# PaullyMac/routest

Measured on AMD Instinct MI355X. Metric: ETA preds/sec (whole node) + p50 /predict latency, 3-layer MLP bf16, higher is better.
Workload: dtype bf16

## Files before the change

### csrc/cch_bindings.cpp

```cpp
#include <torch/extension.h>
#include <ATen/hip/impl/HIPStreamMasqueradingAsCUDA.h>
#include <c10/core/DeviceGuard.h>

#include <chrono>
#include <cmath>
#include <memory>
#include <mutex>
#include <unordered_map>

#include "cch_gpu.h"
#include "ops.h"

namespace py = pybind11;

namespace {

#define CCH_CHECK_HIP(expr)                                                            \
  do {                                                                                 \
    hipError_t _e = (expr);                                                            \
    TORCH_CHECK(_e == hipSuccess, "HIP error in ", #expr, ": ", hipGetErrorString(_e)); \
  } while (0)

hipStream_t stream_of(int dev) { return c10::hip::getCurrentHIPStreamMasqueradingAsCUDA(dev).stream(); }

// ... 267 lines not shown
    o.path = want_path ? path.data_ptr<int>() : nullptr;
    o.max_path = (int)max_path;
    const c10::DeviceGuard guard(src.device());
    std::lock_guard<std::mutex> lk(mu_);
    CCH_CHECK_HIP(g_->route(*m, src.data_ptr<int>(), dst.data_ptr<int>(), (int)Q, o, *sc_, stream_of(dev_)));
    return py::make_tuple(sec, met, st, len, path);
  }

  py::tuple matrix(int64_t key, torch::Tensor pts, torch::Tensor npts) {
    auto m = get(key);
    TORCH_CHECK(pts.is_cuda() && npts.is_cuda() && pts.dim() == 2 && pts.scalar_type() == torch::kInt32 &&
                    npts.scalar_type() == torch::kInt32 && npts.numel() == pts.size(0) && pts.is_contiguous(),
                "pts int32 [R, NM], npts int32 [R] on the router's GPU");
    const int R = (int)pts.size(0), NM = (int)pts.size(1);
    auto of = torch::TensorOptions().dtype(torch::kFloat32).device(torch::kCUDA, dev_);
    auto sec = torch::empty({R, NM, NM}, of), met = torch::empty({R, NM, NM}, of);
    const c10::DeviceGuard guard(pts.device());
    std::lock_guard<std::mutex> lk(mu_);
    CCH_CHECK_HIP(g_->matrix(*m, pts.data_ptr<int>(), npts.data_ptr<int>(), R, NM, sec.data_ptr<float>(),
                             met.data_ptr<float>(), nullptr, *sc_, stream_of(dev_)));
    return py::make_tuple(sec, met);
  }

  py::tuple matrix_rect(int64_t key, torch::Tensor src, torch::Tensor nsrc, torch::Tensor dst, torch::Tensor ndst,
                        int64_t meet) {
    auto m = get(key);
    for (const torch::Tensor* t : {&src, &nsrc, &dst, &ndst})
      TORCH_CHECK(t->is_cuda() && t->device().index() == dev_ && t->scalar_type() == torch::kInt32 && t->is_contiguous(),
                  "src / nsrc / dst / ndst: int32 on the router's GPU");
    TORCH_CHECK(src.dim() == 2 && dst.dim() == 2 && dst.size(0) == src.size(0) && nsrc.numel() == src.size(0) &&
                    ndst.numel() == src.size(0),
                "src [R, SM], dst [R, DM], nsrc [R], ndst [R]");
    const int64_t R = src.size(0), SM = src.size(1), DM = dst.size(1);
    TORCH_CHECK(R * (SM + DM) <= INT32_MAX && R * SM * DM <= INT32_MAX, "matrix_rect: too many chains or cells for one call");
    auto of = torch::TensorOptions().dtype(torch::kFloat32).device(torch::kCUDA, dev_);
    auto sec = torch::empty({R, SM, DM}, of), met = torch::empty({R, SM, DM}, of);
    const c10::DeviceGuard guard(src.device());
    std::lock_guard<std::mutex> lk(mu_);
    CCH_CHECK_HIP(g_->matrix_rect(*m, src.data_ptr<int>(), nsrc.data_ptr<int>(), dst.data_ptr<int>(),
                                  ndst.data_ptr<int>(), (int)R, (int)SM, (int)DM, sec.data_ptr<float>(),
                                  met.data_ptr<float>(), *sc_, stream_of(dev_), (int)meet));
    return py::make_tuple(sec, met);
  }

  py::tuple matrix_keep(int64_t key, torch::Tensor pts, torch::Tensor npts) {
    auto sm = matrix(key, pts, npts);
// ... 107 lines not shown

}

void bind_cch_gpu(py::module& m) {
  py::class_<PyCchGpu>(m, "CchGpu")
      .def(py::init<torch::Tensor, torch::Tensor, torch::Tensor, torch::Tensor, torch::Tensor, torch::Tensor,
                    torch::Tensor, int64_t>(),
           py::arg("indptr"), py::arg("indices"), py::arg("lat"), py::arg("lon"), py::arg("length"),
           py::arg("road_class"), py::arg("base_traffic"), py::arg("device"))
      .def("set_eta", &PyCchGpu::set_eta, py::arg("blob"), py::arg("H"), py::arg("norm"), py::arg("variant") = -1)
      .def("stats", &PyCchGpu::stats)
      .def("metric_for", &PyCchGpu::metric_for, py::arg("weather"), py::arg("congestion"), py::arg("weekhour"),
           py::arg("driver_age") = 35.0, py::arg("pin") = false, py::arg("avoid") = py::none(),
           py::arg("avoid_digest") = 0)
      .def("avoid_mask", &PyCchGpu::avoid_mask, py::arg("blob"))
      .def("unpin", &PyCchGpu::unpin, py::arg("key"))
      .def("pinned", &PyCchGpu::pinned)
      .def("metric_from_costs", &PyCchGpu::metric_from_costs, py::arg("key"), py::arg("cost"))
      .def("costs", &PyCchGpu::costs, py::arg("key"))
      .def("metric_dump", &PyCchGpu::metric_dump, py::arg("key"))
      .def("route", &PyCchGpu::route, py::arg("key"), py::arg("src"), py::arg("dst"), py::arg("max_path") = 4096,
           py::arg("want_path") = true)
      .def("matrix", &PyCchGpu::matrix, py::arg("key"), py::arg("pts"), py::arg("npts"))
      .def("matrix_rect", &PyCchGpu::matrix_rect, py::arg("key"), py::arg("src"), py::arg("nsrc"), py::arg("dst"),
           py::arg("ndst"), py::arg("meet") = 0)
      .def("matrix_keep", &PyCchGpu::matrix_keep, py::arg("key"), py::arg("pts"), py::arg("npts"))
      .def("legs_from_matrix", &PyCchGpu::legs_from_matrix, py::arg("key"), py::arg("tag"), py::arg("pts"), py::arg("r"),
           py::arg("i"), py::arg("j"), py::arg("max_path") = 4096, py::arg("want_path") = true)
      .def("one_to_all", &PyCchGpu::one_to_all, py::arg("key"), py::arg("src"), py::arg("reverse") = false,
           py::arg("fuse") = -1)
      .def("set_capacity", &PyCchGpu::set_capacity)
      .def("set_cache_gb", &PyCchGpu::set_cache_gb, py::arg("gb"))
      .def("set_builder_pacing", &PyCchGpu::set_builder_pacing, py::arg("max_workgroups"), py::arg("always") = false)
      .def("set_unpack_serial", &PyCchGpu::set_unpack_serial, py::arg("on"))
      .def("unpack_serial", &PyCchGpu::unpack_serial)
      .def("request_build", &PyCchGpu::request_build, py::arg("weather"), py::arg("congestion"), py::arg("weekhour"),
           py::arg("driver_age") = 35.0, py::arg("urgent") = true, py::arg("avoid") = py::none(),
           py::arg("avoid_digest") = 0)
      .def("is_cached", &PyCchGpu::is_cached, py::arg("key"))
      .def("ptr", &PyCchGpu::ptr)
      .def("topology_arrays", &PyCchGpu::topology_arrays);
}
```

### csrc/cch_gpu.h

```cpp
#pragma once
#include <hip/hip_runtime.h>

#include <cstdint>
#include <cstdlib>
#include <cstring>
#include <atomic>
#include <chrono>
#include <condition_variable>
#include <deque>
#include <functional>
#include <list>
#include <memory>
#include <mutex>
#include <thread>
#include <unordered_set>
#include <vector>

#include "common.h"
#include "runtime/cch.h"

namespace rt {

struct CchContext {
  int weather = 2, congestion = 1, weekhour = 9;
// ... 22 lines not shown
  int4* b_rec = nullptr;
  int64_t kept_f = 0, kept_b = 0;
  double customize_ms = 0.0, cost_ms = 0.0;
  double basic_ms = 0.0, perfect_ms = 0.0, prune_ms = 0.0;
  double alloc_ms = 0.0, hostcopy_ms = 0.0;
  std::vector<float> host_cost;
  std::shared_ptr<const std::vector<int32_t>> avoid;
  ~CchMetricDev();
};

struct CchScratch {
  float* dist = nullptr;
  int32_t* pred = nullptr;
  int32_t* node = nullptr;
  size_t jobs_cap = 0;
  int32_t* jobs = nullptr;
  int32_t* arcs = nullptr;
  int32_t* narcs = nullptr;
  size_t pairs_cap = 0;
  int32_t* pj = nullptr;
  size_t pj_cap = 0;
  uint64_t chain_tag = 0;
  int chain_nm = 0, chain_r = 0;
  int device = 0;
  std::vector<void*> old;
  ~CchScratch();
  hipError_t ensure(size_t jobs, size_t pairs, int stride, int max_arcs);
};

struct CchAllScratch {
  float* sec = nullptr;
  float* met = nullptr;
  size_t blocks_cap = 0;
  int device = 0;
  std::vector<void*> old;
  ~CchAllScratch();
  hipError_t ensure(size_t blocks, size_t N);
};

struct CustScratch {
  unsigned long long *up64 = nullptr, *dn64 = nullptr;
  uint32_t *pup = nullptr, *pdn = nullptr;
  int32_t *fcnt = nullptr, *bcnt = nullptr;
  void* cub = nullptr;
  size_t cub_bytes = 0;
  void* rec_buf = nullptr;
  float* min_buf = nullptr;
  float* h_stage = nullptr;
  unsigned long long* sup_buf = nullptr;
  int32_t* avoid_dev = nullptr;
// ... 64 lines not shown
  double cache_gb() { std::lock_guard<std::mutex> lk(mu_); return cache_gb_; }
  int capacity() { std::lock_guard<std::mutex> lk(mu_); return capacity_; }
  int64_t metric_bytes() const { return metric_bytes_.load(); }
  int cached() { std::lock_guard<std::mutex> lk(mu_); return (int)cache_.size(); }

  void request_build(const CchContext& c, bool urgent = true);
  void start_builders();
  int add_build_listener(std::function<void(uint64_t, bool)> cb);
  void remove_build_listener(int id);
  struct AsyncStats {
    long long queued = 0, built = 0, failed = 0;
    int pending = 0;
    double build_ms = 0.0, alloc_ms = 0.0, hostcopy_ms = 0.0;
    long long paced = 0;
  };
  AsyncStats async_stats();
  void set_builder_pacing(int n, bool always = false) {
    builder_max_wg_.store(n < 0 ? 0 : n);
    pace_always_.store(always);
  }
  int builder_pacing() const { return builder_max_wg_.load(); }
  void set_unpack_serial(bool on) { unpack_serial_.store(on); }
  bool unpack_serial() const { return unpack_serial_.load(); }
  void note_queries() {
    query_us_.store(std::chrono::duration_cast<std::chrono::microseconds>(
                        std::chrono::steady_clock::now().time_since_epoch()).count(),
                    std::memory_order_relaxed);
  }
  bool serving_now() const {
    const long long now = std::chrono::duration_cast<std::chrono::microseconds>(
                              std::chrono::steady_clock::now().time_since_epoch()).count();
    return now - query_us_.load(std::memory_order_relaxed) < 250000;
  }

  hipError_t route(const CchMetricDev& m, const int* d_src, const int* d_dst, int Q, const CchRouteOut& o,
                   CchScratch& sc, hipStream_t s);
  hipError_t matrix(const CchMetricDev& m, const int* d_pts, const int* d_npts, int R, int NM, float* d_sec,
                    float* d_met, double* d_D64, CchScratch& sc, hipStream_t s);
  hipError_t legs_from_matrix(const CchMetricDev& m, const int* d_src, const int* d_r, const int* d_i, const int* d_j,
                              int Q, uint64_t tag, const CchRouteOut& o, CchScratch& sc, hipStream_t s);
  static constexpr int MAX_ARCS = 1024;
  enum { MEET_AUTO = 0, MEET_RECT = 1, MEET_PAIRS = 2, MEET_NONE = 3 };
  hipError_t matrix_rect(const CchMetricDev& m, const int* d_src, const int* d_nsrc, const int* d_dst,
                         const int* d_ndst, int R, int SM, int DM, float* d_sec, float* d_met, CchScratch& sc,
                         hipStream_t s, int meet = MEET_AUTO);

// ... 1 lines not shown
                        CchAllScratch& sc, hipStream_t s, int fuse = -1);
  static constexpr size_t ALL_SCRATCH_BYTES = 1ull << 30;
  static constexpr int ALL_FUSE_WIDTH = 4;

  static CchMView view(const CchMetricDev& m) {
    return CchMView{m.f_ptr, m.b_ptr, m.f_rec, m.b_rec, m.len_up, m.len_dn, m.sub_up, m.sub_dn, m.cnt_up, m.cnt_dn};
  }
  hipError_t route_multi(const CchMView* d_mv, const int* d_grp, const int* d_src, const int* d_dst, int Q,
                         const CchRouteOut& o, CchScratch& sc, hipStream_t s);
  hipError_t matrix_multi(const CchMView* d_mv, const int* d_row_grp, const int* d_pts, const int* d_npts, int R, int NM,
                          float* d_sec, float* d_met, double* d_D64, CchScratch& sc, hipStream_t s);
  hipError_t legs_from_matrix_multi(const CchMView* d_mv, const int* d_grp, const int* d_src, const int* d_r,
                                    const int* d_i, const int* d_j, int Q, uint64_t tag, const CchRouteOut& o,
                                    CchScratch& sc, hipStream_t s);

 private:
  hipError_t route_impl(const CchMetricDev* m, const CchMView* mv, const int* grp, const int* d_src, const int* d_dst,
                        int Q, const CchRouteOut& o, CchScratch& sc, hipStream_t s);
  hipError_t matrix_impl(const CchMetricDev* m, const CchMView* mv, const int* grp, const int* d_pts, const int* d_npts,
                         int R, int NM, float* d_sec, float* d_met, double* d_D64, CchScratch& sc, hipStream_t s);
  hipError_t legs_impl(const CchMetricDev* m, const CchMView* mv, const int* grp, const int* d_src, const int* d_r,
                       const int* d_i, const int* d_j, int Q, uint64_t tag, const CchRouteOut& o, CchScratch& sc,
                       hipStream_t s);
  hipError_t launch_unpack(const CchMetricDev* m, const CchMView* mv, const int* grp, int Q, const int* d_src,
                           CchScratch& sc, const CchRouteOut& o, hipStream_t s);
  rcch::Topology T_;
  int dev_ = 0;
  int32_t *d_up_ptr = nullptr, *d_up_head = nullptr, *d_arc_lo = nullptr, *d_parent = nullptr, *d_depth = nullptr;
  int32_t *d_rank = nullptr, *d_node = nullptr, *d_edge_arc = nullptr;
  uint8_t* d_edge_dir = nullptr;
  float* d_length = nullptr;
  uint8_t *d_class = nullptr, *d_base_traffic = nullptr;
  int32_t *d_hnodes = nullptr, *d_dnodes = nullptr;
  int32_t* d_dlev_ptr = nullptr;
  int64_t *d_bofs = nullptr, *d_pofs = nullptr;
  std::vector<int64_t> bofs_, pofs_, aofs_;
  std::vector<int> plev_kmax_;
  bool accel_ = false;
  void build_tables();
  void free_tables();
  bool build_triangles(const std::vector<int64_t>& tofs);
  int32_t* d_tri = nullptr;
  int64_t n_tri = 0;
  bool build_tasks(const std::vector<int64_t>& tofs);
  bool build_pull_records(const std::vector<int64_t>& tofs);
  void* d_btask = nullptr;
// ... 51 lines not shown
  int32_t *d_esrc = nullptr, *d_edst = nullptr, *d_qx = nullptr, *d_qy = nullptr;
  std::atomic<uint64_t> tag_ctr_{0};
  void builder_loop(int idx);
  void start_builders_locked();
  void notify_built(uint64_t key, bool ok);
  std::vector<std::thread> bths_;
  std::mutex bmu_;
  std::condition_variable bcv_;
  std::deque<CchContext> bq_;
  std::unordered_set<uint64_t> bpending_;
  bool bstop_ = false;
  std::mutex lmu_;
  std::vector<std::pair<int, std::function<void(uint64_t, bool)>>> listeners_;
  int next_listener_ = 1;
  std::atomic<long long> n_bqueued_{0}, n_bbuilt_{0}, n_bfailed_{0};
  std::atomic<long long> us_build_{0}, us_alloc_{0}, us_hostcopy_{0};
  std::atomic<long long> query_us_{-(1LL << 40)};
  std::atomic<bool> pace_always_{false};
  std::atomic<long long> n_paced_{0};
  std::atomic<int> builder_max_wg_{[] {
    const char* v = std::getenv("ROUTEST_CCH_BUILDER_MAX_WG");
    return v ? std::max(0, std::atoi(v)) : -1;
  }()};
  std::atomic<bool> unpack_serial_{[] {
    const char* v = std::getenv("ROUTEST_CCH_UNPACK");
    return v != nullptr && std::strcmp(v, "serial") == 0;
  }()};
};

}
```

### csrc/cch_query.hip

```cpp
#include "cch_dev.h"
#include "cch_gpu.h"

namespace rt {

using namespace cchd;

namespace {

constexpr int SWEEP_AHEAD = 3;
constexpr int SWEEP_RECS = 4;

typedef int sweep_v4i __attribute__((ext_vector_type(4)));

struct SweepRecs {
  sweep_v4i r[SWEEP_RECS];
};

__device__ __forceinline__ SweepRecs sweep_fetch(const int4* __restrict__ rec, int pb, int pe, int i, int L, int lane) {
  SweepRecs v;
  const int ii = i < 63 ? i : 63;
  const int b = __shfl(pb, ii);
  const int e = i < L ? __shfl(pe, ii) : b;
#pragma unroll
  for (int k = 0; k < SWEEP_RECS; ++k) {
    const int idx = b + lane + 64 * k;
    const int4* p = rec + (idx < e ? idx : 0);
    asm volatile("global_load_dwordx4 %0, %1, off" : "=v"(v.r[k]) : "v"(p));
  }
  return v;
}

template <int NEWER>
__device__ __forceinline__ void sweep_wait(SweepRecs& q) {
  static_assert(NEWER * SWEEP_RECS <= 63, "vmcnt range");
  asm volatile("s_waitcnt vmcnt(%4)" : "+v"(q.r[0]), "+v"(q.r[1]), "+v"(q.r[2]), "+v"(q.r[3]) : "n"(NEWER * SWEEP_RECS));
}

__device__ __forceinline__ void sweep_relax(float* sd, int32_t* sp, float dx, int w, int hd, int arc) {
  const float nd = dx + __int_as_float(w);
  if (nd < sd[hd]) {
    sd[hd] = nd;
    sp[hd] = arc;
  }
}

__global__ __launch_bounds__(64) void sweep_kernel(const int32_t* __restrict__ jobs, int J,
                                                   const int32_t* __restrict__ parent,
                                                   const int32_t* __restrict__ depth, int N,
                                                   const int32_t* __restrict__ f_ptr, const int4* __restrict__ f_rec,
                                                   const int32_t* __restrict__ b_ptr, const int4* __restrict__ b_rec,
                                                   int stride, float* __restrict__ out_dist,
                                                   int32_t* __restrict__ out_pred, int32_t* __restrict__ out_node,
                                                   const CchMView* __restrict__ mv, const int32_t* __restrict__ grp,
                                                   int gdiv) {
  extern __shared__ unsigned char smem[];
  float* sd = reinterpret_cast<float*>(smem);
  int32_t* sp = reinterpret_cast<int32_t*>(smem + (size_t)stride * 4);
  const int j = blockIdx.x;
  if (j >= J) return;
  const int lane = threadIdx.x;
  const int code = jobs[j];
  if (code < 0) return;
  const int r = code >> 1;
  const bool fwd = (code & 1) == 0;
  if (mv != nullptr) {
    const CchMView& v = mv[grp[j / gdiv]];
    f_ptr = v.f_ptr;
    f_rec = v.f_rec;
    b_ptr = v.b_ptr;
    b_rec = v.b_rec;
  }
  const int32_t* __restrict__ ptr = fwd ? f_ptr : b_ptr;
  const int4* __restrict__ rec = fwd ? f_rec : b_rec;
  const int D = depth[r];
  for (int d = lane; d <= D; d += 64) {
    sd[d] = F_INF;
    sp[d] = -1;
  }
  __syncthreads();
  if (lane == 0) sd[D] = 0.f;
  __syncthreads();
  const size_t base = (size_t)j * stride;
  int x = r, d = D;
  int cand = x + lane;
  int par = cand < N ? parent[cand] : -2;
  int pb = cand < N ? ptr[cand] : 0;
  int pe = cand < N ? ptr[cand + 1] : 0;
  while (x >= 0 && d >= 0) {
    const unsigned long long cont = __ballot(cand < N && par == cand + 1);
    int L = (~cont == 0ull) ? 64 : (__builtin_ctzll(~cont) + 1);
    if (L > d + 1) L = d + 1;
    const int next = __shfl(par, L - 1);
    if (lane < L) out_node[base + (d - lane)] = x + lane;
    const int ncand = next + lane;
    const bool nin = next >= 0 && ncand < N;
    const int npar = nin ? parent[ncand] : -2;
    const int npb = nin ? ptr[ncand] : 0;
    const int npe = nin ? ptr[ncand + 1] : 0;
    auto node = [&](int i, const SweepRecs& q) {
      if (i >= L) return;
      const float dx = sd[d - i];
      if (dx < F_INF) {
        const int b = __shfl(pb, i), e = __shfl(pe, i);
#pragma unroll
        for (int k = 0; k < SWEEP_RECS; ++k)
          if (b + lane + 64 * k < e) sweep_relax(sd, sp, dx, q.r[k].x, q.r[k].y, q.r[k].z);
        for (int k = b + 64 * SWEEP_RECS + lane; k < e; k += 64) {
          const int4 rc = rec[k];
          sweep_relax(sd, sp, dx, rc.x, rc.y, rc.z);
        }
        __syncthreads();
      }
    };
    SweepRecs qa = sweep_fetch(rec, pb, pe, 0, L, lane);
    SweepRecs qb = sweep_fetch(rec, pb, pe, 1, L, lane);
    SweepRecs qc = sweep_fetch(rec, pb, pe, 2, L, lane);
    for (int i = 0; i < L; i += 4) {
      SweepRecs qd = sweep_fetch(rec, pb, pe, i + 3, L, lane);
      sweep_wait<3>(qa);
      node(i, qa);
      qa = sweep_fetch(rec, pb, pe, i + 4, L, lane);
      sweep_wait<3>(qb);
      node(i + 1, qb);
      qb = sweep_fetch(rec, pb, pe, i + 5, L, lane);
      sweep_wait<3>(qc);
      node(i + 2, qc);
      qc = sweep_fetch(rec, pb, pe, i + 6, L, lane);
      sweep_wait<3>(qd);
      node(i + 3, qd);
// ... 4 lines not shown
    x = next;
    d -= L;
    cand = ncand;
    par = npar;
    pb = npb;
    pe = npe;
  }
  __syncthreads();
  for (int dd = lane; dd <= D; dd += 64) {
    out_dist[base + dd] = sd[dd];
    out_pred[base + dd] = sp[dd];
  }
}

__global__ __launch_bounds__(64) void meet_kernel(int P, const int32_t* __restrict__ pjf, const int32_t* __restrict__ pjb,
                                                  int jf0, int jb0, const int32_t* __restrict__ jobs, int stride,
                                                  const float* __restrict__ sdist, const int32_t* __restrict__ spred,
                                                  const int32_t* __restrict__ snode, const int32_t* __restrict__ depth,
                                                  const int32_t* __restrict__ arc_lo, const float* __restrict__ len_up,
                                                  const float* __restrict__ len_dn, float* __restrict__ out_sec,
                                                  float* __restrict__ out_met, int* __restrict__ out_status,
                                                  int32_t* __restrict__ arcs, int32_t* __restrict__ narcs, int max_arcs,
                                                  const CchMView* __restrict__ mv, const int32_t* __restrict__ grp,
                                                  int gdiv) {
  __shared__ int32_t fw[4096];
  const int q = blockIdx.x;
  if (q >= P) return;
  const int lane = threadIdx.x;
  if (mv != nullptr) {
    const CchMView& v = mv[grp[q / gdiv]];
    len_up = v.len_up;
    len_dn = v.len_dn;
  }
  const int jf = pjf ? pjf[q] : jf0 + 2 * q;
  const int jb = pjb ? pjb[q] : jb0 + 2 * q;
  if (jobs[jf] < 0 || jobs[jb] < 0) {
    if (threadIdx.x == 0) {
      if (out_sec) out_sec[q] = -1.f;
      if (out_met) out_met[q] = -1.f;
      if (out_status) out_status[q] = 1;
      if (narcs) narcs[q] = 0;
    }
    return;
  }
  const int s = jobs[jf] >> 1, t = jobs[jb] >> 1;
  const int ds = depth[s], dt = depth[t];
  const size_t bf = (size_t)jf * stride, bb = (size_t)jb * stride;
  int status = 1;
  float best = F_INF;
  int bestd = -1;
  if (snode[bf] == snode[bb]) {
    int lo = 0, hi = ds < dt ? ds : dt;
    while (lo < hi) {
      const int mid = (lo + hi + 1) >> 1;
      if (snode[bf + mid] == snode[bb + mid]) lo = mid;
      else hi = mid - 1;
    }
    const int L = lo;
// ... 307 lines not shown
                                 const int* __restrict__ ndst, int R, int SM, int DM, const int32_t* __restrict__ rank,
                                 int N, int32_t* __restrict__ jobs) {
  const long long g = blockIdx.x * (long long)blockDim.x + threadIdx.x;
  const int W = SM + DM;
  if (g >= (long long)R * W) return;
  const int r = (int)(g / W), k = (int)(g % W);
  const bool fwd = k < SM;
  const int i = fwd ? k : k - SM;
  if (i >= (fwd ? nsrc[r] : ndst[r])) {
    jobs[g] = -1;
    return;
  }
  int v = fwd ? src[(size_t)r * SM + i] : dst[(size_t)r * DM + i];
  if (v < 0 || v >= N) v = 0;
  jobs[g] = (rank[v] << 1) | (fwd ? 0 : 1);
}

constexpr int MEET_TILE = 64;
constexpr int MEET_THREADS = 256;
__global__ __launch_bounds__(MEET_THREADS) void meet_rect_kernel(
    int SM, int DM, const int* __restrict__ nsrc, const int* __restrict__ ndst, const int32_t* __restrict__ jobs,
    int stride, const float* __restrict__ sdist, const int32_t* __restrict__ spred, const int32_t* __restrict__ snode,
    const int32_t* __restrict__ depth, const int32_t* __restrict__ arc_lo, const float* __restrict__ len_up,
    const float* __restrict__ len_dn, float* __restrict__ out_sec, float* __restrict__ out_met) {
  extern __shared__ unsigned char smem[];
  int32_t* fn = reinterpret_cast<int32_t*>(smem);
  float* fd = reinterpret_cast<float*>(smem + (size_t)stride * 4);
  int32_t* fp = reinterpret_cast<int32_t*>(smem + (size_t)stride * 8);
  __shared__ float s_best[MEET_TILE];
  __shared__ int s_bestd[MEET_TILE];
  const int tid = threadIdx.x;
  const int ntile = (DM + MEET_TILE - 1) / MEET_TILE;
  const int tile = blockIdx.x % ntile;
  const int i = (blockIdx.x / ntile) % SM;
  const int r = blockIdx.x / (ntile * SM);
  const int j0 = tile * MEET_TILE;
  const int nj = min(MEET_TILE, DM - j0);
  const int nv = min(nj, ndst[r] - j0);
  const size_t cell = ((size_t)r * SM + i) * DM + j0;
  if (i >= nsrc[r] || nv <= 0) {
    if (tid < nj) {
      out_sec[cell + tid] = 0.f;
      out_met[cell + tid] = 0.f;
    }
    return;
  }
  const size_t jrow = (size_t)r * (SM + DM);
  const int s = jobs[jrow + i] >> 1;
  const int ds = depth[s];
  const size_t bf = (jrow + i) * stride;
  for (int d = tid; d <= ds; d += MEET_THREADS) {
    fn[d] = snode[bf + d];
    fd[d] = sdist[bf + d];
    fp[d] = spred[bf + d];
  }
  __syncthreads();
  const int lane = tid & 63;
  for (int p = tid >> 6; p < nv; p += MEET_THREADS / 64) {
    const size_t jb = jrow + SM + j0 + p;
    const int t = jobs[jb] >> 1;
    const int dt = depth[t];
    const size_t bb = jb * stride;
    float best = F_INF;
    int bestd = -1;
    if (fn[0] == snode[bb]) {
      int lo = 0, hi = ds < dt ? ds : dt;
      while (lo < hi) {
        const int mid = (lo + hi + 1) >> 1;
        if (fn[mid] == snode[bb + mid]) lo = mid;
        else hi = mid - 1;
      }
      const int L = lo;
      for (int d = lane; d <= L; d += 64) {
        const float v = fd[d] + sdist[bb + d];
        if (v < best || (v == best && d > bestd)) {
          best = v;
          bestd = d;
        }
      }
#pragma unroll
      for (int o = 32; o >= 1; o >>= 1) {
        const float ov = __shfl_xor(best, o);
        const int od = __shfl_xor(bestd, o);
        if (ov < best || (ov == best && od > bestd)) {
          best = ov;
          bestd = od;
        }
      }
    }
    if (lane == 0) {
      s_best[p] = best;
      s_bestd[p] = bestd;
    }
  }
  __syncthreads();
  if (tid >= nj) return;
  float sec = 0.f, met = 0.f;
  if (tid < nv) {
    const size_t jb = jrow + SM + j0 + tid;
    const int t = jobs[jb] >> 1;
    if (t != s) {
      sec = s_best[tid];
      if (sec < F_INF) {
        const int dt = depth[t];
        const size_t bb = jb * stride;
        const int bestd = s_bestd[tid];
        for (int slot = bestd; slot != ds;) {
          const int a = fp[slot];
          met += len_up[a];
          slot = depth[arc_lo[a]];
        }
        for (int slot = bestd; slot != dt;) {
          const int a = spred[bb + slot];
          met += len_dn[a];
          slot = depth[arc_lo[a]];
        }
      } else {
        sec = met = F_INF;
      }
    }
  }
  out_sec[cell + tid] = sec;
  out_met[cell + tid] = met;
}

__global__ void rect_pairs_kernel(int R, int SM, int DM, int32_t* __restrict__ pjf, int32_t* __restrict__ pjb) {
  const long long g = blockIdx.x * (long long)blockDim.x + threadIdx.x;
  if (g >= (long long)R * SM * DM) return;
// ... 1 lines not shown
  const int rem = (int)(g % ((long long)SM * DM));
  pjf[g] = r * (SM + DM) + rem / DM;
  pjb[g] = r * (SM + DM) + SM + rem % DM;
}

__global__ void rect_out_kernel(const int* __restrict__ nsrc, const int* __restrict__ ndst, int R, int SM, int DM,
                                const int32_t* __restrict__ jobs, float* __restrict__ sec, float* __restrict__ met) {
  const long long g = blockIdx.x * (long long)blockDim.x + threadIdx.x;
  if (g >= (long long)R * SM * DM) return;
  const int r = (int)(g / ((long long)SM * DM));
  const int rem = (int)(g % ((long long)SM * DM));
  const int i = rem / DM, j = rem % DM;
  float s = sec[g], m = met[g];
  const size_t jrow = (size_t)r * (SM + DM);
  if (i >= nsrc[r] || j >= ndst[r] || (jobs[jrow + i] >> 1) == (jobs[jrow + SM + j] >> 1)) s = m = 0.f;
  else {
    if (s < 0.f) s = F_INF;
    if (m < 0.f) m = F_INF;
  }
  sec[g] = s;
  met[g] = m;
}

}

CchScratch::~CchScratch() {
  int cur = 0;
  (void)hipGetDevice(&cur);
  (void)hipSetDevice(device);
  dfree(dist);
  dfree(pred);
  dfree(node);
  dfree(jobs);
  dfree(arcs);
  dfree(narcs);
  dfree(pj);
  for (void* p : old) (void)hipFree(p);
  (void)hipSetDevice(cur);
}

hipError_t CchScratch::ensure(size_t J, size_t P, int stride, int max_arcs) {
  hipError_t e = hipSuccess;
  auto retire = [&](auto*& p) {
    if (p) old.push_back((void*)p);
    p = nullptr;
  };
  if (J > jobs_cap) {
    retire(dist);
    retire(pred);
    retire(node);
    retire(jobs);
    const size_t cap = std::max(J, jobs_cap * 3 / 2);
    if ((e = dmalloc(dist, cap * stride)) != hipSuccess) return e;
    if ((e = dmalloc(pred, cap * stride)) != hipSuccess) return e;
    if ((e = dmalloc(node, cap * stride)) != hipSuccess) return e;
    if ((e = dmalloc(jobs, cap)) != hipSuccess) return e;
    jobs_cap = cap;
  }
  if (P > pairs_cap) {
    retire(arcs);
    retire(narcs);
    const size_t cap = std::max(P, pairs_cap * 3 / 2);
    if ((e = dmalloc(arcs, cap * (size_t)max_arcs)) != hipSuccess) return e;
    if ((e = dmalloc(narcs, cap)) != hipSuccess) return e;
    pairs_cap = cap;
  }
  return e;
}

hipError_t CchGpu::launch_unpack(const CchMetricDev* m, const CchMView* mv, const int* grp, int Q, const int* d_src,
                                 CchScratch& sc, const CchRouteOut& o, hipStream_t s) {
  const bool serial_only = unpack_serial();
  const int32_t* sub_up = m ? m->sub_up : nullptr;
  const int32_t* sub_dn = m ? m->sub_dn : nullptr;
  if (!serial_only) {
    constexpr int G = 64 / UNPACK_LANES;
    hipLaunchKernelGGL(unpack_coop_kernel, dim3((Q + G - 1) / G), dim3(64), 0, s, Q, d_src, sc.arcs, sc.narcs, MAX_ARCS,
                       sub_up, sub_dn, m ? m->cnt_up : nullptr, m ? m->cnt_dn : nullptr, d_arc_lo, d_up_head, d_node,
                       o.status, o.len, o.path, o.max_path, o.edges, mv, grp);
    hipError_t e = hipGetLastError();
    if (e != hipSuccess) return e;
  }
  hipLaunchKernelGGL(unpack_kernel, dim3(blocks_for(Q, 64)), dim3(64), 0, s, Q, d_src, sc.arcs, sc.narcs, MAX_ARCS,
                     sub_up, sub_dn, d_arc_lo, d_up_head, d_node, o.status, o.len, o.path, o.max_path,
                     serial_only ? -1 : UNPACK_MAX_ARCS, o.edges, mv, grp);
  return hipGetLastError();
}

hipError_t CchGpu::route_impl(const CchMetricDev* m, const CchMView* mv, const int* grp, const int* d_src,
                              const int* d_dst, int Q, const CchRouteOut& o, CchScratch& sc, hipStream_t s) {
  if (Q <= 0) return hipSuccess;
  const int S = stride();
  sc.device = dev_;
  sc.chain_tag = 0;
  hipError_t e = sc.ensure((size_t)2 * Q, (size_t)Q, S, MAX_ARCS);
  if (e != hipSuccess) return e;
  hipLaunchKernelGGL(route_jobs_kernel, dim3(blocks_for(Q, 256)), dim3(256), 0, s, d_src, d_dst, Q, d_rank, T_.N,
                     sc.jobs);
  hipLaunchKernelGGL(sweep_kernel, dim3(2 * Q), dim3(64), (size_t)S * 8, s, sc.jobs, 2 * Q, d_parent, d_depth, T_.N,
                     m ? m->f_ptr : nullptr, m ? m->f_rec : nullptr, m ? m->b_ptr : nullptr, m ? m->b_rec : nullptr, S,
                     sc.dist, sc.pred, sc.node, mv, grp, 2);
  if ((e = hipGetLastError()) != hipSuccess) return e;
  hipLaunchKernelGGL(meet_kernel, dim3(Q), dim3(64), 0, s, Q, nullptr, nullptr, 0, 1, sc.jobs, S, sc.dist, sc.pred,
                     sc.node, d_depth, d_arc_lo, m ? m->len_up : nullptr, m ? m->len_dn : nullptr, o.sec, o.metres,
                     o.status, o.path ? sc.arcs : nullptr, o.path ? sc.narcs : nullptr, MAX_ARCS, mv, grp, 1);
  if ((e = hipGetLastError()) != hipSuccess) return e;
  if (o.path != nullptr) e = launch_unpack(m, mv, grp, Q, d_src, sc, o, s);
  return e;
}

hipError_t CchGpu::route(const CchMetricDev& m, const int* d_src, const int* d_dst, int Q, const CchRouteOut& o,
                         CchScratch& sc, hipStream_t s) {
  return route_impl(&m, nullptr, nullptr, d_src, d_dst, Q, o, sc, s);
}

hipError_t CchGpu::route_multi(const CchMView* d_mv, const int* d_grp, const int* d_src, const int* d_dst, int Q,
                               const CchRouteOut& o, CchScratch& sc, hipStream_t s) {
  if (d_mv == nullptr || d_grp == nullptr) return hipErrorInvalidValue;
  return route_impl(nullptr, d_mv, d_grp, d_src, d_dst, Q, o, sc, s);
}

hipError_t CchGpu::matrix_impl(const CchMetricDev* m, const CchMView* mv, const int* grp, const int* d_pts,
                               const int* d_npts, int R, int NM, float* d_sec, float* d_met, double* d_D64,
                               CchScratch& sc, hipStream_t s) {
  if (R <= 0 || NM <= 0) return hipSuccess;
  if (d_sec == nullptr || d_met == nullptr) return hipErrorInvalidValue;
  const int S = stride();
  sc.device = dev_;
  const size_t J = (size_t)R * NM * 2, P = (size_t)R * NM * NM;
  hipError_t e = sc.ensure(J, (P * 2 + MAX_ARCS - 1) / MAX_ARCS + 1, S, MAX_ARCS);
  if (e != hipSuccess) return e;
  int32_t* pjf = sc.arcs;
  int32_t* pjb = sc.arcs + P;
  float* sec = d_sec;
  float* met = d_met;
  hipLaunchKernelGGL(matrix_jobs_kernel, dim3(blocks_for((long long)R * NM, 256)), dim3(256), 0, s, d_pts, d_npts, R, NM,
                     d_rank, T_.N, sc.jobs);
  hipLaunchKernelGGL(matrix_pairs_kernel, dim3(blocks_for((long long)P, 256)), dim3(256), 0, s, d_npts, R, NM, pjf, pjb);
  hipLaunchKernelGGL(sweep_kernel, dim3((unsigned)J), dim3(64), (size_t)S * 8, s, sc.jobs, (int)J, d_parent, d_depth,
                     T_.N, m ? m->f_ptr : nullptr, m ? m->f_rec : nullptr, m ? m->b_ptr : nullptr,
                     m ? m->b_rec : nullptr, S, sc.dist, sc.pred, sc.node, mv, grp, 2 * NM);
  if ((e = hipGetLastError()) != hipSuccess) return e;
  hipLaunchKernelGGL(meet_kernel, dim3((unsigned)P), dim3(64), 0, s, (int)P, pjf, pjb, 0, 0, sc.jobs, S, sc.dist,
                     sc.pred, sc.node, d_depth, d_arc_lo, m ? m->len_up : nullptr, m ? m->len_dn : nullptr, sec, met,
                     nullptr, nullptr, nullptr, MAX_ARCS, mv, grp, NM * NM);
  if ((e = hipGetLastError()) != hipSuccess) return e;
  hipLaunchKernelGGL(matrix_out_kernel, dim3(blocks_for((long long)P, 256)), dim3(256), 0, s, d_npts, R, NM, sec, met,
                     d_D64);
  e = hipGetLastError();
  sc.chain_tag = e == hipSuccess ? ++tag_ctr_ : 0;
  sc.chain_nm = NM;
  sc.chain_r = R;
  return e;
}

hipError_t CchGpu::matrix(const CchMetricDev& m, const int* d_pts, const int* d_npts, int R, int NM, float* d_sec,
                          float* d_met, double* d_D64, CchScratch& sc, hipStream_t s) {
  return matrix_impl(&m, nullptr, nullptr, d_pts, d_npts, R, NM, d_sec, d_met, d_D64, sc, s);
}

hipError_t CchGpu::matrix_multi(const CchMView* d_mv, const int* d_row_grp, const int* d_pts, const int* d_npts, int R,
                                int NM, float* d_sec, float* d_met, double* d_D64, CchScratch& sc, hipStream_t s) {
  if (d_mv == nullptr || d_row_grp == nullptr) return hipErrorInvalidValue;
  return matrix_impl(nullptr, d_mv, d_row_grp, d_pts, d_npts, R, NM, d_sec, d_met, d_D64, sc, s);
}

hipError_t CchGpu::matrix_rect(const CchMetricDev& m, const int* d_src, const int* d_nsrc, const int* d_dst,
                               const int* d_ndst, int R, int SM, int DM, float* d_sec, float* d_met, CchScratch& sc,
                               hipStream_t s, int meet) {
  if (R <= 0 || SM <= 0 || DM <= 0) return hipSuccess;
  if (d_sec == nullptr || d_met == nullptr || meet < MEET_AUTO || meet > MEET_NONE) return hipErrorInvalidValue;
  const int S = stride();
  const size_t J = (size_t)R * ((size_t)SM + DM), P = (size_t)R * SM * DM;
  if (J > (size_t)INT32_MAX || P > (size_t)INT32_MAX) return hipErrorInvalidValue;
  const size_t lds = (size_t)S * 12;
  const bool fits = lds + MEET_TILE * 8 <= 64 * 1024;
  if (meet == MEET_RECT && !fits) return hipErrorInvalidValue;
  if (meet == MEET_AUTO) meet = fits ? MEET_RECT : MEET_PAIRS;
  sc.device = dev_;
  sc.chain_tag = 0;
  hipError_t e = sc.ensure(J, meet == MEET_PAIRS ? (P * 2 + MAX_ARCS - 1) / MAX_ARCS + 1 : 0, S, MAX_ARCS);
  if (e != hipSuccess) return e;
  hipLaunchKernelGGL(rect_jobs_kernel, dim3(blocks_for((long long)J, 256)), dim3(256), 0, s, d_src, d_nsrc, d_dst,
                     d_ndst, R, SM, DM, d_rank, T_.N, sc.jobs);
  hipLaunchKernelGGL(sweep_kernel, dim3((unsigned)J), dim3(64), (size_t)S * 8, s, sc.jobs, (int)J, d_parent, d_depth,
                     T_.N, m.f_ptr, m.f_rec, m.b_ptr, m.b_rec, S, sc.dist, sc.pred, sc.node, nullptr, nullptr, 1);
  if ((e = hipGetLastError()) != hipSuccess) return e;
  if (meet == MEET_RECT) {
    const size_t blocks = (size_t)R * SM * ((DM + MEET_TILE - 1) / MEET_TILE);
    hipLaunchKernelGGL(meet_rect_kernel, dim3((unsigned)blocks), dim3(MEET_THREADS), lds, s, SM, DM, d_nsrc, d_ndst,
                       sc.jobs, S, sc.dist, sc.pred, sc.node, d_depth, d_arc_lo, m.len_up, m.len_dn, d_sec, d_met);
  } else if (meet == MEET_PAIRS) {
    int32_t* pjf = sc.arcs;
    int32_t* pjb = sc.arcs + P;
    hipLaunchKernelGGL(rect_pairs_kernel, dim3(blocks_for((long long)P, 256)), dim3(256), 0, s, R, SM, DM, pjf, pjb);
    hipLaunchKernelGGL(meet_kernel, dim3((unsigned)P), dim3(64), 0, s, (int)P, pjf, pjb, 0, 0, sc.jobs, S, sc.dist,
                       sc.pred, sc.node, d_depth, d_arc_lo, m.len_up, m.len_dn, d_sec, d_met, nullptr, nullptr, nullptr,
                       MAX_ARCS, nullptr, nullptr, 1);
    if ((e = hipGetLastError()) != hipSuccess) return e;
    hipLaunchKernelGGL(rect_out_kernel, dim3(blocks_for((long long)P, 256)), dim3(256), 0, s, d_nsrc, d_ndst, R, SM, DM,
                       sc.jobs, d_sec, d_met);
  }
  return hipGetLastError();
}

hipError_t CchGpu::legs_impl(const CchMetricDev* m, const CchMView* mv, const int* grp, const int* d_src,
                             const int* d_r, const int* d_i, const int* d_j, int Q, uint64_t tag, const CchRouteOut& o,
                             CchScratch& sc, hipStream_t s) {
  if (Q <= 0) return hipSuccess;
  if (tag == 0 || tag != sc.chain_tag) return hipErrorInvalidValue;
  const int S = stride();
  hipError_t e = sc.ensure(0, (size_t)Q, S, MAX_ARCS);
  if (e != hipSuccess) return e;
  if ((size_t)Q > sc.pj_cap) {
    if (sc.pj) sc.old.push_back((void*)sc.pj);
    sc.pj = nullptr;
    const size_t cap = std::max((size_t)Q, sc.pj_cap * 3 / 2);
    if ((e = dmalloc(sc.pj, 2 * cap)) != hipSuccess) return e;
    sc.pj_cap = cap;
  }
  int32_t* pjf = sc.pj;
  int32_t* pjb = sc.pj + sc.pj_cap;
  hipLaunchKernelGGL(leg_pairs_kernel, dim3(blocks_for(Q, 256)), dim3(256), 0, s, sc.chain_nm, d_r, d_i, d_j, Q,
                     sc.chain_r, pjf, pjb);
  if ((e = hipGetLastError()) != hipSuccess) return e;
  hipLaunchKernelGGL(meet_kernel, dim3(Q), dim3(64), 0, s, Q, pjf, pjb, 0, 0, sc.jobs, S, sc.dist, sc.pred, sc.node,
                     d_depth, d_arc_lo, m ? m->len_up : nullptr, m ? m->len_dn : nullptr, o.sec, o.metres, o.status,
                     o.path ? sc.arcs : nullptr, o.path ? sc.narcs : nullptr, MAX_ARCS, mv, grp, 1);
  if ((e = hipGetLastError()) != hipSuccess) return e;
  if (o.path != nullptr) e = launch_unpack(m, mv, grp, Q, d_src, sc, o, s);
  return e;
}

hipError_t CchGpu::legs_from_matrix(const CchMetricDev& m, const int* d_src, const int* d_r, const int* d_i,
                                    const int* d_j, int Q, uint64_t tag, const CchRouteOut& o, CchScratch& sc,
                                    hipStream_t s) {
  return legs_impl(&m, nullptr, nullptr, d_src, d_r, d_i, d_j, Q, tag, o, sc, s);
}

hipError_t CchGpu::legs_from_matrix_multi(const CchMView* d_mv, const int* d_grp, const int* d_src, const int* d_r,
                                          const int* d_i, const int* d_j, int Q, uint64_t tag, const CchRouteOut& o,
                                          CchScratch& sc, hipStream_t s) {
  if (d_mv == nullptr || d_grp == nullptr) return hipErrorInvalidValue;
  return legs_impl(nullptr, d_mv, d_grp, d_src, d_r, d_i, d_j, Q, tag, o, sc, s);
}

}
```

Baseline: 6.517 billion.

## Deduplicate identical CCH sweep jobs via GPU hash table and skip diagonal meets

Adds a GPU hash-based canonicalisation step that maps duplicate (metric group, node, direction) sweep jobs to a single representative, so sweep_kernel runs only the unique jobs and meet kernels read from the canonical slot. Diagonal matrix pairs are short-circuited to zero, and the sweep relax loop switches to readlane plus grouped relax variants chosen by arc count. It also adds matrix_multi and debug bindings. The cost is two extra small kernels plus a memset per call, and more indirection in the meet kernels.

```diff
diff --git a/csrc/cch_bindings.cpp b/csrc/cch_bindings.cpp
--- a/csrc/cch_bindings.cpp
+++ b/csrc/cch_bindings.cpp
@@ -313,6 +313,50 @@
     return py::make_tuple(sec, met);
   }
 
+  py::tuple matrix_multi(std::vector<int64_t> keys, torch::Tensor row_group, torch::Tensor pts, torch::Tensor npts) {
+    TORCH_CHECK(!keys.empty(), "matrix_multi: no metric");
+    TORCH_CHECK(pts.is_cuda() && npts.is_cuda() && row_group.is_cuda() && pts.dim() == 2 &&
+                    pts.scalar_type() == torch::kInt32 && npts.scalar_type() == torch::kInt32 &&
+                    row_group.scalar_type() == torch::kInt32 && npts.numel() == pts.size(0) &&
+                    row_group.numel() == pts.size(0) && pts.is_contiguous() && row_group.is_contiguous() &&
+                    npts.is_contiguous(),
+                "pts int32 [R, NM], npts int32 [R], row_group int32 [R] on the router's GPU");
+    const int R = (int)pts.size(0), NM = (int)pts.size(1);
+    if (R > 0)
+      TORCH_CHECK(row_group.min().item<int>() >= 0 && row_group.max().item<int>() < (int)keys.size(),
+                  "row_group out of range");
+    std::vector<std::shared_ptr<rt::CchMetricDev>> ms;
+    std::vector<rt::CchMView> views;
+    for (int64_t k : keys) {
+      ms.push_back(get(k));
+      views.push_back(rt::CchGpu::view(*ms.back()));
+    }
+    const int64_t vbytes = (int64_t)(views.size() * sizeof(rt::CchMView));
+    auto hv = torch::empty({vbytes}, torch::kUInt8);
+    std::memcpy(hv.data_ptr(), views.data(), (size_t)vbytes);
+    auto of = torch::TensorOptions().dtype(torch::kFloat32).device(torch::kCUDA, dev_);
+    auto sec = torch::empty({R, NM, NM}, of), met = torch::empty({R, NM, NM}, of);
+    const c10::DeviceGuard guard(pts.device());
+    auto dv = hv.to(pts.device());
+    std::lock_guard<std::mutex> lk(mu_);
+    CCH_CHECK_HIP(g_->matrix_multi(reinterpret_cast<const rt::CchMView*>(dv.data_ptr()), row_group.data_ptr<int>(),
+                                   pts.data_ptr<int>(), npts.data_ptr<int>(), R, NM, sec.data_ptr<float>(),
+                                   met.data_ptr<float>(), nullptr, *sc_, stream_of(dev_)));
+    CCH_CHECK_HIP(hipStreamSynchronize(stream_of(dev_)));
+    return py::make_tuple(sec, met);
+  }
+
+  torch::Tensor last_canon() {
+    std::lock_guard<std::mutex> lk(mu_);
+    const c10::DeviceGuard guard(torch::Device(torch::kCUDA, dev_));
+    std::vector<int32_t> h;
+    CCH_CHECK_HIP(sc_->canon_host(h, stream_of(dev_)));
+    auto out = torch::empty({(int64_t)h.size()}, torch::kInt32);
+    if (!h.empty()) std::memcpy(out.data_ptr<int32_t>(), h.data(), h.size() * 4);
+    return out;
+  }
+  bool chain_dedup() const { return g_->chain_dedup(); }
+
   py::tuple matrix_rect(int64_t key, torch::Tensor src, torch::Tensor nsrc, torch::Tensor dst, torch::Tensor ndst,
                         int64_t meet) {
     auto m = get(key);
@@ -466,6 +510,10 @@
       .def("route", &PyCchGpu::route, py::arg("key"), py::arg("src"), py::arg("dst"), py::arg("max_path") = 4096,
            py::arg("want_path") = true)
       .def("matrix", &PyCchGpu::matrix, py::arg("key"), py::arg("pts"), py::arg("npts"))
+      .def("matrix_multi", &PyCchGpu::matrix_multi, py::arg("keys"), py::arg("row_group"), py::arg("pts"),
+           py::arg("npts"))
+      .def("last_canon", &PyCchGpu::last_canon)
+      .def("chain_dedup", &PyCchGpu::chain_dedup)
       .def("matrix_rect", &PyCchGpu::matrix_rect, py::arg("key"), py::arg("src"), py::arg("nsrc"), py::arg("dst"),
            py::arg("ndst"), py::arg("meet") = 0)
       .def("matrix_keep", &PyCchGpu::matrix_keep, py::arg("key"), py::arg("pts"), py::arg("npts"))
diff --git a/csrc/cch_gpu.h b/csrc/cch_gpu.h
--- a/csrc/cch_gpu.h
+++ b/csrc/cch_gpu.h
@@ -68,10 +68,16 @@
   size_t pj_cap = 0;
   uint64_t chain_tag = 0;
   int chain_nm = 0, chain_r = 0;
+  int32_t* canon = nullptr;
+  uint32_t* ctab = nullptr;
+  size_t ctab_cap = 0;
+  size_t canon_n = 0;
+  bool canon_on = false;
   int device = 0;
   std::vector<void*> old;
   ~CchScratch();
   hipError_t ensure(size_t jobs, size_t pairs, int stride, int max_arcs);
+  hipError_t canon_host(std::vector<int32_t>& out, hipStream_t s) const;
 };
 
 struct CchAllScratch {
@@ -182,6 +188,7 @@
   int builder_pacing() const { return builder_max_wg_.load(); }
   void set_unpack_serial(bool on) { unpack_serial_.store(on); }
   bool unpack_serial() const { return unpack_serial_.load(); }
+  bool chain_dedup() const { return dedup_; }
   void note_queries() {
     query_us_.store(std::chrono::duration_cast<std::chrono::microseconds>(
                         std::chrono::steady_clock::now().time_since_epoch()).count(),
@@ -229,6 +236,8 @@
   hipError_t legs_impl(const CchMetricDev* m, const CchMView* mv, const int* grp, const int* d_src, const int* d_r,
                        const int* d_i, const int* d_j, int Q, uint64_t tag, const CchRouteOut& o, CchScratch& sc,
                        hipStream_t s);
+  hipError_t build_canon(CchScratch& sc, size_t J, const CchMView* mv, const int* grp, int gdiv, hipStream_t s,
+                         const int32_t** canon);
   hipError_t launch_unpack(const CchMetricDev* m, const CchMView* mv, const int* grp, int Q, const int* d_src,
                            CchScratch& sc, const CchRouteOut& o, hipStream_t s);
   rcch::Topology T_;
@@ -326,6 +335,10 @@
     const char* v = std::getenv("ROUTEST_CCH_BUILDER_MAX_WG");
     return v ? std::max(0, std::atoi(v)) : -1;
   }()};
+  const bool dedup_ = [] {
+    const char* v = std::getenv("ROUTEST_CCH_DEDUP");
+    return v == nullptr || std::strcmp(v, "0") != 0;
+  }();
   std::atomic<bool> unpack_serial_{[] {
     const char* v = std::getenv("ROUTEST_CCH_UNPACK");
     return v != nullptr && std::strcmp(v, "serial") == 0;
diff --git a/csrc/cch_query.hip b/csrc/cch_query.hip
--- a/csrc/cch_query.hip
+++ b/csrc/cch_query.hip
@@ -14,17 +14,18 @@
 
 struct SweepRecs {
   sweep_v4i r[SWEEP_RECS];
+  int b, e;
 };
 
 __device__ __forceinline__ SweepRecs sweep_fetch(const int4* __restrict__ rec, int pb, int pe, int i, int L, int lane) {
   SweepRecs v;
   const int ii = i < 63 ? i : 63;
-  const int b = __shfl(pb, ii);
-  const int e = i < L ? __shfl(pe, ii) : b;
+  v.b = __builtin_amdgcn_readlane(pb, ii);
+  v.e = i < L ? __builtin_amdgcn_readlane(pe, ii) : v.b;
 #pragma unroll
   for (int k = 0; k < SWEEP_RECS; ++k) {
-    const int idx = b + lane + 64 * k;
-    const int4* p = rec + (idx < e ? idx : 0);
+    const int idx = v.b + lane + 64 * k;
+    const int4* p = rec + (idx < v.e ? idx : 0);
     asm volatile("global_load_dwordx4 %0, %1, off" : "=v"(v.r[k]) : "v"(p));
   }
   return v;
@@ -41,6 +42,21 @@
   if (nd < sd[hd]) {
     sd[hd] = nd;
     sp[hd] = arc;
+  }
+}
+
+template <int G>
+__device__ __forceinline__ void sweep_relax_groups(float* sd, int32_t* sp, float dx, const SweepRecs& q, int n) {
+  float old[G];
+#pragma unroll
+  for (int k = 0; k < G; ++k) old[k] = sd[q.r[k].y];
+#pragma unroll
+  for (int k = 0; k < G; ++k) {
+    const float nd = dx + __int_as_float(q.r[k].x);
+    if (64 * k < n && nd < old[k]) {
+      sd[q.r[k].y] = nd;
+      sp[q.r[k].y] = q.r[k].z;
+    }
   }
 }
 
@@ -52,7 +68,7 @@
                                                    int stride, float* __restrict__ out_dist,
                                                    int32_t* __restrict__ out_pred, int32_t* __restrict__ out_node,
                                                    const CchMView* __restrict__ mv, const int32_t* __restrict__ grp,
-                                                   int gdiv) {
+                                                   int gdiv, const int32_t* __restrict__ canon) {
   extern __shared__ unsigned char smem[];
   float* sd = reinterpret_cast<float*>(smem);
   int32_t* sp = reinterpret_cast<int32_t*>(smem + (size_t)stride * 4);
@@ -61,6 +77,7 @@
   const int lane = threadIdx.x;
   const int code = jobs[j];
   if (code < 0) return;
+  if (canon != nullptr && canon[j] != j) return;
   const int r = code >> 1;
   const bool fwd = (code & 1) == 0;
   if (mv != nullptr) {
@@ -98,13 +115,14 @@
     const int npb = nin ? ptr[ncand] : 0;
     const int npe = nin ? ptr[ncand + 1] : 0;
     auto node = [&](int i, const SweepRecs& q) {
-      if (i >= L) return;
+      const int b = q.b, e = q.e;
+      if (i >= L || e <= b) return;
       const float dx = sd[d - i];
       if (dx < F_INF) {
-        const int b = __shfl(pb, i), e = __shfl(pe, i);
-#pragma unroll
-        for (int k = 0; k < SWEEP_RECS; ++k)
-          if (b + lane + 64 * k < e) sweep_relax(sd, sp, dx, q.r[k].x, q.r[k].y, q.r[k].z);
+        const int n = e - b - lane;
+        if (e - b <= 64) sweep_relax_groups<1>(sd, sp, dx, q, n);
+        else if (e - b <= 128) sweep_relax_groups<2>(sd, sp, dx, q, n);
+        else sweep_relax_groups<SWEEP_RECS>(sd, sp, dx, q, n);
         for (int k = b + 64 * SWEEP_RECS + lane; k < e; k += 64) {
           const int4 rc = rec[k];
           sweep_relax(sd, sp, dx, rc.x, rc.y, rc.z);
@@ -155,7 +173,7 @@
                                                   float* __restrict__ out_met, int* __restrict__ out_status,
                                                   int32_t* __restrict__ arcs, int32_t* __restrict__ narcs, int max_arcs,
                                                   const CchMView* __restrict__ mv, const int32_t* __restrict__ grp,
-                                                  int gdiv) {
+                                                  int gdiv, const int32_t* __restrict__ canon, int skip_diag) {
   __shared__ int32_t fw[4096];
   const int q = blockIdx.x;
   if (q >= P) return;
@@ -165,8 +183,19 @@
     len_up = v.len_up;
     len_dn = v.len_dn;
   }
-  const int jf = pjf ? pjf[q] : jf0 + 2 * q;
-  const int jb = pjb ? pjb[q] : jb0 + 2 * q;
+  int jf = pjf ? pjf[q] : jf0 + 2 * q;
+  int jb = pjb ? pjb[q] : jb0 + 2 * q;
+  if (skip_diag && (jf >> 1) == (jb >> 1)) {
+    if (threadIdx.x == 0) {
+      out_sec[q] = 0.f;
+      out_met[q] = 0.f;
+    }
+    return;
+  }
+  if (canon != nullptr) {
+    jf = canon[jf];
+    jb = canon[jb];
+  }
   if (jobs[jf] < 0 || jobs[jb] < 0) {
     if (threadIdx.x == 0) {
       if (out_sec) out_sec[q] = -1.f;
@@ -520,7 +549,8 @@
     int SM, int DM, const int* __restrict__ nsrc, const int* __restrict__ ndst, const int32_t* __restrict__ jobs,
     int stride, const float* __restrict__ sdist, const int32_t* __restrict__ spred, const int32_t* __restrict__ snode,
     const int32_t* __restrict__ depth, const int32_t* __restrict__ arc_lo, const float* __restrict__ len_up,
-    const float* __restrict__ len_dn, float* __restrict__ out_sec, float* __restrict__ out_met) {
+    const float* __restrict__ len_dn, float* __restrict__ out_sec, float* __restrict__ out_met,
+    const int32_t* __restrict__ canon) {
   extern __shared__ unsigned char smem[];
   int32_t* fn = reinterpret_cast<int32_t*>(smem);
   float* fd = reinterpret_cast<float*>(smem + (size_t)stride * 4);
@@ -546,7 +576,7 @@
   const size_t jrow = (size_t)r * (SM + DM);
   const int s = jobs[jrow + i] >> 1;
   const int ds = depth[s];
-  const size_t bf = (jrow + i) * stride;
+  const size_t bf = (size_t)(canon ? canon[jrow + i] : jrow + i) * stride;
   for (int d = tid; d <= ds; d += MEET_THREADS) {
     fn[d] = snode[bf + d];
     fd[d] = sdist[bf + d];
@@ -558,7 +588,7 @@
     const size_t jb = jrow + SM + j0 + p;
     const int t = jobs[jb] >> 1;
     const int dt = depth[t];
-    const size_t bb = jb * stride;
+    const size_t bb = (size_t)(canon ? canon[jb] : jb) * stride;
     float best = F_INF;
     int bestd = -1;
     if (fn[0] == snode[bb]) {
@@ -601,7 +631,7 @@
       sec = s_best[tid];
       if (sec < F_INF) {
         const int dt = depth[t];
-        const size_t bb = jb * stride;
+        const size_t bb = (size_t)(canon ? canon[jb] : jb) * stride;
         const int bestd = s_bestd[tid];
         for (int slot = bestd; slot != ds;) {
           const int a = fp[slot];
@@ -649,6 +679,37 @@
   met[g] = m;
 }
 
+constexpr unsigned long long CANON_EMPTY = ~0ull;
+
+__global__ void canon_insert_kernel(const int32_t* __restrict__ jobs, int J, const int32_t* __restrict__ grp, int gdiv,
+                                    unsigned long long* __restrict__ keys, unsigned int* __restrict__ vals,
+                                    unsigned int mask, int32_t* __restrict__ canon) {
+  const int j = blockIdx.x * blockDim.x + threadIdx.x;
+  if (j >= J) return;
+  const int code = jobs[j];
+  if (code < 0) {
+    canon[j] = j;
+    return;
+  }
+  const unsigned int g = grp != nullptr ? (unsigned int)grp[j / gdiv] : 0u;
+  const unsigned long long key = ((unsigned long long)g << 32) | (unsigned int)code;
+  unsigned int h = (unsigned int)((key * 0x9E3779B97F4A7C15ull) >> 32) & mask;
+  for (;;) {
+    const unsigned long long was = atomicCAS(&keys[h], CANON_EMPTY, key);
+    if (was == CANON_EMPTY || was == key) break;
+    h = (h + 1) & mask;
+  }
+  atomicMin(&vals[h], (unsigned int)j);
+  canon[j] = (int32_t)h;
+}
+
+__global__ void canon_read_kernel(const int32_t* __restrict__ jobs, int J, const unsigned int* __restrict__ vals,
+                                  int32_t* __restrict__ canon) {
+  const int j = blockIdx.x * blockDim.x + threadIdx.x;
+  if (j >= J || jobs[j] < 0) return;
+  canon[j] = (int32_t)vals[canon[j]];
+}
+
 }
 
 CchScratch::~CchScratch() {
@@ -662,6 +723,8 @@
   dfree(arcs);
   dfree(narcs);
   dfree(pj);
+  dfree(canon);
+  dfree(ctab);
   for (void* p : old) (void)hipFree(p);
   (void)hipSetDevice(cur);
 }
@@ -677,11 +740,14 @@
     retire(pred);
     retire(node);
     retire(jobs);
+    retire(canon);
+    canon_on = false;
     const size_t cap = std::max(J, jobs_cap * 3 / 2);
     if ((e = dmalloc(dist, cap * stride)) != hipSuccess) return e;
     if ((e = dmalloc(pred, cap * stride)) != hipSuccess) return e;
     if ((e = dmalloc(node, cap * stride)) != hipSuccess) return e;
     if ((e = dmalloc(jobs, cap)) != hipSuccess) return e;
+    if ((e = dmalloc(canon, cap)) != hipSuccess) return e;
     jobs_cap = cap;
   }
   if (P > pairs_cap) {
@@ -693,6 +759,46 @@
     pairs_cap = cap;
   }
   return e;
+}
+
+hipError_t CchScratch::canon_host(std::vector<int32_t>& out, hipStream_t s) const {
+  out.resize(canon_n);
+  if (!canon_on) {
+    for (size_t j = 0; j < canon_n; ++j) out[j] = (int32_t)j;
+    return hipSuccess;
+  }
+  if (canon_n == 0) return hipSuccess;
+  hipError_t e = hipMemcpyAsync(out.data(), canon, canon_n * sizeof(int32_t), hipMemcpyDeviceToHost, s);
+  return e != hipSuccess ? e : hipStreamSynchronize(s);
+}
+
+hipError_t CchGpu::build_canon(CchScratch& sc, size_t J, const CchMView* mv, const int* grp, int gdiv, hipStream_t s,
+                               const int32_t** canon) {
+  *canon = nullptr;
+  sc.canon_n = J;
+  sc.canon_on = false;
+  if (!dedup_ || J == 0) return hipSuccess;
+  size_t T = 64;
+  while (T < 2 * J) T <<= 1;
+  hipError_t e = hipSuccess;
+  if (T > sc.ctab_cap) {
+    if (sc.ctab) sc.old.push_back((void*)sc.ctab);
+    sc.ctab = nullptr;
+    sc.ctab_cap = 0;
+    if ((e = dmalloc(sc.ctab, 3 * T)) != hipSuccess) return e;
+    sc.ctab_cap = T;
+  }
+  if ((e = hipMemsetAsync(sc.ctab, 0xFF, 3 * T * sizeof(uint32_t), s)) != hipSuccess) return e;
+  unsigned long long* keys = reinterpret_cast<unsigned long long*>(sc.ctab);
+  unsigned int* vals = sc.ctab + 2 * T;
+  hipLaunchKernelGGL(canon_insert_kernel, dim3(blocks_for((long long)J, 256)), dim3(256), 0, s, sc.jobs, (int)J,
+                     mv != nullptr ? grp : nullptr, gdiv, keys, vals, (unsigned int)(T - 1), sc.canon);
+  hipLaunchKernelGGL(canon_read_kernel, dim3(blocks_for((long long)J, 256)), dim3(256), 0, s, sc.jobs, (int)J, vals,
+                     sc.canon);
+  if ((e = hipGetLastError()) != hipSuccess) return e;
+  sc.canon_on = true;
+  *canon = sc.canon;
+  return hipSuccess;
 }
 
 hipError_t CchGpu::launch_unpack(const CchMetricDev* m, const CchMView* mv, const int* grp, int Q, const int* d_src,
@@ -724,13 +830,15 @@
   if (e != hipSuccess) return e;
   hipLaunchKernelGGL(route_jobs_kernel, dim3(blocks_for(Q, 256)), dim3(256), 0, s, d_src, d_dst, Q, d_rank, T_.N,
                      sc.jobs);
+  const int32_t* canon = nullptr;
+  if ((e = build_canon(sc, (size_t)2 * Q, mv, grp, 2, s, &canon)) != hipSuccess) return e;
   hipLaunchKernelGGL(sweep_kernel, dim3(2 * Q), dim3(64), (size_t)S * 8, s, sc.jobs, 2 * Q, d_parent, d_depth, T_.N,
                      m ? m->f_ptr : nullptr, m ? m->f_rec : nullptr, m ? m->b_ptr : nullptr, m ? m->b_rec : nullptr, S,
-                     sc.dist, sc.pred, sc.node, mv, grp, 2);
+                     sc.dist, sc.pred, sc.node, mv, grp, 2, canon);
   if ((e = hipGetLastError()) != hipSuccess) return e;
   hipLaunchKernelGGL(meet_kernel, dim3(Q), dim3(64), 0, s, Q, nullptr, nullptr, 0, 1, sc.jobs, S, sc.dist, sc.pred,
                      sc.node, d_depth, d_arc_lo, m ? m->len_up : nullptr, m ? m->len_dn : nullptr, o.sec, o.metres,
-                     o.status, o.path ? sc.arcs : nullptr, o.path ? sc.narcs : nullptr, MAX_ARCS, mv, grp, 1);
+                     o.status, o.path ? sc.arcs : nullptr, o.path ? sc.narcs : nullptr, MAX_ARCS, mv, grp, 1, canon, 0);
   if ((e = hipGetLastError()) != hipSuccess) return e;
   if (o.path != nullptr) e = launch_unpack(m, mv, grp, Q, d_src, sc, o, s);
   return e;
@@ -764,13 +872,15 @@
   hipLaunchKernelGGL(matrix_jobs_kernel, dim3(blocks_for((long long)R * NM, 256)), dim3(256), 0, s, d_pts, d_npts, R, NM,
                      d_rank, T_.N, sc.jobs);
   hipLaunchKernelGGL(matrix_pairs_kernel, dim3(blocks_for((long long)P, 256)), dim3(256), 0, s, d_npts, R, NM, pjf, pjb);
+  const int32_t* canon = nullptr;
+  if ((e = build_canon(sc, J, mv, grp, 2 * NM, s, &canon)) != hipSuccess) return e;
   hipLaunchKernelGGL(sweep_kernel, dim3((unsigned)J), dim3(64), (size_t)S * 8, s, sc.jobs, (int)J, d_parent, d_depth,
                      T_.N, m ? m->f_ptr : nullptr, m ? m->f_rec : nullptr, m ? m->b_ptr : nullptr,
-                     m ? m->b_rec : nullptr, S, sc.dist, sc.pred, sc.node, mv, grp, 2 * NM);
+                     m ? m->b_rec : nullptr, S, sc.dist, sc.pred, sc.node, mv, grp, 2 * NM, canon);
   if ((e = hipGetLastError()) != hipSuccess) return e;
   hipLaunchKernelGGL(meet_kernel, dim3((unsigned)P), dim3(64), 0, s, (int)P, pjf, pjb, 0, 0, sc.jobs, S, sc.dist,
                      sc.pred, sc.node, d_depth, d_arc_lo, m ? m->len_up : nullptr, m ? m->len_dn : nullptr, sec, met,
-                     nullptr, nullptr, nullptr, MAX_ARCS, mv, grp, NM * NM);
+                     nullptr, nullptr, nullptr, MAX_ARCS, mv, grp, NM * NM, canon, 1);
   if ((e = hipGetLastError()) != hipSuccess) return e;
   hipLaunchKernelGGL(matrix_out_kernel, dim3(blocks_for((long long)P, 256)), dim3(256), 0, s, d_npts, R, NM, sec, met,
                      d_D64);
@@ -810,20 +920,23 @@
   if (e != hipSuccess) return e;
   hipLaunchKernelGGL(rect_jobs_kernel, dim3(blocks_for((long long)J, 256)), dim3(256), 0, s, d_src, d_nsrc, d_dst,
                      d_ndst, R, SM, DM, d_rank, T_.N, sc.jobs);
+  const int32_t* canon = nullptr;
+  if ((e = build_canon(sc, J, nullptr, nullptr, 1, s, &canon)) != hipSuccess) return e;
   hipLaunchKernelGGL(sweep_kernel, dim3((unsigned)J), dim3(64), (size_t)S * 8, s, sc.jobs, (int)J, d_parent, d_depth,
-                     T_.N, m.f_ptr, m.f_rec, m.b_ptr, m.b_rec, S, sc.dist, sc.pred, sc.node, nullptr, nullptr, 1);
+                     T_.N, m.f_ptr, m.f_rec, m.b_ptr, m.b_rec, S, sc.dist, sc.pred, sc.node, nullptr, nullptr, 1, canon);
   if ((e = hipGetLastError()) != hipSuccess) return e;
   if (meet == MEET_RECT) {
     const size_t blocks = (size_t)R * SM * ((DM + MEET_TILE - 1) / MEET_TILE);
     hipLaunchKernelGGL(meet_rect_kernel, dim3((unsigned)blocks), dim3(MEET_THREADS), lds, s, SM, DM, d_nsrc, d_ndst,
-                       sc.jobs, S, sc.dist, sc.pred, sc.node, d_depth, d_arc_lo, m.len_up, m.len_dn, d_sec, d_met);
+                       sc.jobs, S, sc.dist, sc.pred, sc.node, d_depth, d_arc_lo, m.len_up, m.len_dn, d_sec, d_met,
+                       canon);
   } else if (meet == MEET_PAIRS) {
     int32_t* pjf = sc.arcs;
     int32_t* pjb = sc.arcs + P;
     hipLaunchKernelGGL(rect_pairs_kernel, dim3(blocks_for((long long)P, 256)), dim3(256), 0, s, R, SM, DM, pjf, pjb);
     hipLaunchKernelGGL(meet_kernel, dim3((unsigned)P), dim3(64), 0, s, (int)P, pjf, pjb, 0, 0, sc.jobs, S, sc.dist,
                        sc.pred, sc.node, d_depth, d_arc_lo, m.len_up, m.len_dn, d_sec, d_met, nullptr, nullptr, nullptr,
-                       MAX_ARCS, nullptr, nullptr, 1);
+                       MAX_ARCS, nullptr, nullptr, 1, canon, 0);
     if ((e = hipGetLastError()) != hipSuccess) return e;
     hipLaunchKernelGGL(rect_out_kernel, dim3(blocks_for((long long)P, 256)), dim3(256), 0, s, d_nsrc, d_ndst, R, SM, DM,
                        sc.jobs, d_sec, d_met);
@@ -853,7 +966,8 @@
   if ((e = hipGetLastError()) != hipSuccess) return e;
   hipLaunchKernelGGL(meet_kernel, dim3(Q), dim3(64), 0, s, Q, pjf, pjb, 0, 0, sc.jobs, S, sc.dist, sc.pred, sc.node,
                      d_depth, d_arc_lo, m ? m->len_up : nullptr, m ? m->len_dn : nullptr, o.sec, o.metres, o.status,
-                     o.path ? sc.arcs : nullptr, o.path ? sc.narcs : nullptr, MAX_ARCS, mv, grp, 1);
+                     o.path ? sc.arcs : nullptr, o.path ? sc.narcs : nullptr, MAX_ARCS, mv, grp, 1,
+                     sc.canon_on ? sc.canon : nullptr, 0);
   if ((e = hipGetLastError()) != hipSuccess) return e;
   if (o.path != nullptr) e = launch_unpack(m, mv, grp, Q, d_src, sc, o, s);
   return e;
```

New measurement: 6.519 billion, median of 2. No clear change (+0.0%).
